# gchhablani/multilingual-image-captioning

Hardware: AMD Instinct MI355X
Metric: train images/sec, ViT-B/32+mBART-50 (bf16 train step, batch 64/GPU, 224x224, seq_len 64) (higher is better)
Workload: dtype bf16

## Files before the change

### include/mic_hip.h

```cpp
#ifndef MIC_HIP_H
#define MIC_HIP_H
#include <stdint.h>
#ifdef __cplusplus
extern "C" {
#endif

#define MIC_OK 0
#define MIC_EINVAL (-1)
#define MIC_ELAUNCH (-2)

#define MIC_BF16 0
#define MIC_F32 1
#define MIC_FP8 2
#define MIC_E4M3 0
#define MIC_E5M2 1

#define MIC_ACT_NONE 0
#define MIC_ACT_GELU_ERF 1
#define MIC_ACT_GELU_TANH 2
#define MIC_ACT_QUICK_GELU 3

int mic_version(void);
const char* mic_last_error(void);

// ... 125 lines not shown
int mic_ce_rows_tiles(int dtype, int rows, int V, const void* logits, int ld, const float* rowstat, int stat_ld,
                      const int32_t* labels, float* row_lse, float* row_loss, void* stream);
int mic_ce_reduce(int rows, const float* row_loss, const int32_t* mask, float* loss_out, float* denom_out,
                  void* stream);
int mic_ce_bwd(int dtype, int rows, int V, int Vpad, void* logits, int ld, const int32_t* labels,
               const int32_t* mask, float label_smoothing, const float* row_lse, const float* denom,
               float loss_scale, void* stream);
int mic_ce_bwd_q8(int rows, int V, int Vpad, const void* logits, int ld, const int32_t* labels, const int32_t* mask,
                  float label_smoothing, const float* row_lse, const float* denom, float loss_scale, const mic_fp8_out* q8,
                  float* colsum, float* label_coef, void* stream);
int mic_head_label_terms(int rows, int width, const int32_t* labels, const float* coef, const void* E, int lde, const void* h, int ldh,
                         float* dx_slab, int ldx, float* dE, int ldde, void* stream);
int mic_ce_bwd_t(int rows, int V, int Vpad, void* logits, int ld, const int32_t* labels, const int32_t* mask, float label_smoothing,
                 const float* row_lse, const float* denom, float loss_scale, void* dlogits_t, int ld_t, int rows_pad, float* colsum,
                 void* stream);
int mic_transpose_bf16(int rows, int rows_pad, int cols, const void* src, int ld_src, void* dst, int ld_dst, void* stream);

int mic_colsum(int dtype, int rows, int cols, const void* x, int ld, float* out, int accumulate, void* stream);
typedef struct { const void* x; float* out; int rows, cols, ld; } mic_colsum_item;
int mic_colsum_grouped(int dtype, const mic_colsum_item* items, int count, void* stream);
typedef struct { const void* x; float* out; const float* scale_inv; int rows, cols, ld, fmt; } mic_colsum_q8_item;
int mic_colsum_q8_grouped(const mic_colsum_q8_item* items, int count, void* stream);
int mic_dropout_mask(uint8_t* out, int64_t n, float p, uint32_t seed, void* stream);
int mic_cast(int src_dtype, int dst_dtype, const void* src, void* dst, int64_t n, void* stream);
int mic_zero(void* p, int64_t bytes, void* stream);
int mic_stream_create_cu_masked(int first_cu, int n_cus, void** stream);
int mic_stream_destroy(void* stream);
int mic_comm_emulate(const void* src, void* dst, int64_t bytes, float micros, int blocks, void* stream);
int mic_copy_rows(int dtype, int n, int width, const void* src, int ld_src, const int32_t* src_idx, void* dst, int ld_dst,
                  const int32_t* dst_idx, void* stream);
// ... 54 lines not shown
```

### multilingual-image-captioning_amd/_lib.py

```python
from __future__ import annotations

import ctypes as C
import os

_HERE = os.path.dirname(os.path.abspath(__file__))
LIB_PATH = os.path.join(_HERE, "libmic_hip.so")

MIC_BF16, MIC_F32, MIC_FP8 = 0, 1, 2
MIC_E4M3, MIC_E5M2 = 0, 1
ACT_NONE, ACT_GELU_ERF, ACT_GELU_TANH, ACT_QUICK_GELU = 0, 1, 2, 3
ACT_IDS = {"none": 0, None: 0, "gelu": 1, "erf": 1, "gelu_erf": 1, "tanh": 2, "gelu_tanh": 2, "gelu_new": 2, "quick_gelu": 3}


class MicError(RuntimeError):
    pass


class GemmArgs(C.Structure):
    _fields_ = [
        ("dtype", C.c_int), ("c_dtype", C.c_int), ("M", C.c_int), ("N", C.c_int), ("K", C.c_int),
        ("a_kmajor", C.c_int), ("b_kmajor", C.c_int),
        ("A", C.c_void_p), ("lda", C.c_int), ("B", C.c_void_p), ("ldb", C.c_int), ("C", C.c_void_p), ("ldc", C.c_int),
        ("bias", C.c_void_p), ("act", C.c_int), ("Zout", C.c_void_p), ("ldz", C.c_int), ("Zin", C.c_void_p),
        ("dact", C.c_int), ("R", C.c_void_p), ("ldr", C.c_int), ("accumulate", C.c_int), ("dropout_p", C.c_float),
# ... 84 lines not shown
    "mic_attn_decode": ([_i, _i, _i, _i, _i, _p, _i, _p, _p, _i, _p, _i, _p, _i, _p], C.c_int),
    "mic_kv_append": ([_i, _i, _i, _i, _i, _p, _i, _p, _i, _p, _p, _p], C.c_int),
    "mic_im2col": ([_i, _i, _i, _i, _p, _p, _i, _i, _p], C.c_int),
    "mic_vit_assemble": ([_i, _i, _i, _i, _p, _i, _p, _p, _p, _p], C.c_int),
    "mic_vit_assemble_bwd": ([_i, _i, _i, _i, _p, _p, _i, _p, _p, _p], C.c_int),
    "mic_embed_fwd": ([_i, _i, _i, _p, _p, _p, _p, _f, _p, _p], C.c_int),
    "mic_embed_bwd": ([_i, _i, _i, _p, _p, _p, _f, _p, _p, _p], C.c_int),
    "mic_embed_rows_add_det": ([_i, _i, _i, _i, _p, _p, _f, _p, _p, _p], C.c_int),
    "mic_embed_rows_add_det_ws": ([_i], C.c_int64),
    "mic_ce_rows": ([_i, _i, _i, _p, _i, _p, _p, _f, _p, _p, _p], C.c_int),
    "mic_ce_rows_tiles": ([_i, _i, _i, _p, _i, _p, _i, _p, _p, _p, _p], C.c_int),
    "mic_row_topk_tiles": ([_i, _i, _i, _p, _i, _p, _i, _i, _i, _i, _i, _p, _p, _p, _p], C.c_int),
    "mic_ce_reduce": ([_i, _p, _p, _p, _p, _p], C.c_int),
    "mic_ce_bwd": ([_i, _i, _i, _i, _p, _i, _p, _p, _f, _p, _p, _f, _p], C.c_int),
    "mic_ce_bwd_t": ([_i, _i, _i, _p, _i, _p, _p, _f, _p, _p, _f, _p, _i, _i, _p, _p], C.c_int),
    "mic_ce_bwd_q8": ([_i, _i, _i, _p, _i, _p, _p, _f, _p, _p, _f, C.POINTER(Fp8Out), _p, _p, _p], C.c_int),
    "mic_head_label_terms": ([_i, _i, _p, _p, _p, _i, _p, _i, _p, _i, _p, _i, _p], C.c_int),
    "mic_transpose_bf16": ([_i, _i, _i, _p, _i, _p, _i, _p], C.c_int),
    "mic_colsum": ([_i, _i, _i, _p, _i, _p, _i, _p], C.c_int),
    "mic_colsum_grouped": ([_i, C.POINTER(ColsumItem), _i, _p], C.c_int),
    "mic_dropout_mask": ([_p, _i64, _f, _u32, _p], C.c_int),
    "mic_cast": ([_i, _i, _p, _p, _i64, _p], C.c_int),
    "mic_zero": ([_p, _i64, _p], C.c_int),
    "mic_stream_create_cu_masked": ([_i, _i, C.POINTER(C.c_void_p)], C.c_int),
    "mic_stream_destroy": ([_p], C.c_int),
    "mic_copy_rows": ([_i, _i, _i, _p, _i, _p, _p, _i, _p, _p], C.c_int),
    "mic_cast2d": ([_i, _i, _i, _i, _p, _i, _p, _i, _p], C.c_int),
    "mic_adamw": ([_i64, _p, _p, _p, _p, _p, _p, C.c_double, C.c_double, C.c_double, C.c_double, _f, _p], C.c_int),
    "mic_adamw_rows": ([_i64, _i, _p, _i, _p, _p, _p, _p, _p, _p, C.c_double, C.c_double, C.c_double, C.c_double, _f, _p], C.c_int),
    "mic_row_flags": ([_p, _i, _p, _i, _p], C.c_int),
# ... 30 lines not shown
```

### multilingual-image-captioning_amd/csrc/elementwise.hip

```cpp
#include "common.h"
#include <stdarg.h>
#include <type_traits>

static thread_local char g_err[512] = "";
void mic_set_error(const char* fmt, ...) {
  va_list ap;
  va_start(ap, fmt);
  vsnprintf(g_err, sizeof(g_err), fmt, ap);
  va_end(ap);
}
extern "C" const char* mic_last_error(void) { return g_err; }
extern "C" int mic_version(void) { return 1; }

template <typename F>
static int dispatch_t(int dtype, F&& f) {
  if (dtype == MIC_BF16) f((uint16_t*)nullptr);
  else if (dtype == MIC_F32) f((float*)nullptr);
  else { mic_set_error("bad dtype %d", dtype); return MIC_EINVAL; }
  hipError_t e = hipGetLastError();
  if (e != hipSuccess) { mic_set_error("launch failed: %s", hipGetErrorString(e)); return MIC_ELAUNCH; }
  return MIC_OK;
}
#define TYPE_OF(tag) typename std::remove_pointer<decltype(tag)>::type

// ... 497 lines not shown
                          float loss_scale, void* stream) {
  MIC_CHECK(rows > 0 && V > 1 && Vpad >= V && Vpad % 8 == 0 && ld >= Vpad && logits && labels && mask && row_lse && denom, "mic_ce_bwd: bad args");
  return dispatch_t(dtype, [&](auto* tag) {
    using T = TYPE_OF(tag);
    hipLaunchKernelGGL(ce_bwd_kernel<T>, dim3(rows), dim3(256), 0, (hipStream_t)stream, V, Vpad, (T*)logits, ld, labels, mask, label_smoothing, row_lse, denom, loss_scale);
  });
}

struct TransposeArgs {
  const uint16_t* src; uint16_t* src_rw; int ld_src;
  uint16_t* dst; int ld_dst;
  int rows, cols;
  int V; const int32_t* labels; const int32_t* mask; float ls; const float* row_lse; const float* denom; float loss_scale;
  float* colsum;
};
template <int OP>
__global__ __launch_bounds__(256) void tile_transpose_kernel(TransposeArgs a) {
  __shared__ __attribute__((aligned(16))) char img[64 * 1024];
  const int tid = threadIdx.x, lane = tid & 63, wave = tid >> 6;
  const int c0 = blockIdx.x * 512, r0 = blockIdx.y * 64;
  const int col = c0 + lane * 8;
  const bool col_ok = col < a.cols;
  uint4 q[16];
#pragma unroll
  for (int rr = 0; rr < 16; ++rr) {
    const int row = r0 + wave * 16 + rr;
    q[rr] = make_uint4(0u, 0u, 0u, 0u);
    if (row < a.rows && col_ok) q[rr] = *reinterpret_cast<const uint4*>(a.src + (size_t)row * a.ld_src + col);
  }
  float inv_denom = 0.f;
  if constexpr (OP == 1) inv_denom = a.loss_scale / a.denom[0];
#pragma unroll
  for (int rr = 0; rr < 16; ++rr) {
// ... 63 lines not shown
}
extern "C" int mic_ce_bwd_t(int rows, int V, int Vpad, void* logits, int ld, const int32_t* labels, const int32_t* mask,
                            float label_smoothing, const float* row_lse, const float* denom, float loss_scale, void* dlogits_t,
                            int ld_t, int rows_pad, float* colsum, void* stream) {
  if (rows_pad <= 0) rows_pad = (rows + 63) / 64 * 64;
  MIC_CHECK(rows_pad >= rows && rows_pad % 64 == 0, "mic_ce_bwd_t: rows_pad >= rows, a multiple of 64");
  MIC_CHECK(rows > 0 && V > 1 && Vpad >= V && Vpad % 8 == 0 && ld >= Vpad && ld % 8 == 0 && logits && labels && mask && row_lse && denom && dlogits_t,
            "mic_ce_bwd_t: bad args");
  MIC_CHECK(ld_t >= rows_pad && ld_t % 8 == 0 && ((uintptr_t)logits & 15) == 0 && ((uintptr_t)dlogits_t & 15) == 0,
            "mic_ce_bwd_t: ld_t >= rows rounded up to 64, ld_t %% 8 == 0, 16-B aligned operands");
  TransposeArgs a{};
  a.src = (const uint16_t*)logits; a.src_rw = (uint16_t*)logits; a.ld_src = ld; a.dst = (uint16_t*)dlogits_t; a.ld_dst = ld_t;
  a.rows = rows; a.cols = Vpad; a.V = V; a.labels = labels; a.mask = mask; a.ls = label_smoothing; a.row_lse = row_lse; a.denom = denom;
  a.loss_scale = loss_scale; a.colsum = colsum;
  hipLaunchKernelGGL(tile_transpose_kernel<1>, dim3((Vpad + 511) / 512, rows_pad / 64), dim3(256), 0, (hipStream_t)stream, a);
  MIC_LAUNCH_CHECK();
  return MIC_OK;
}

struct CeQ8Args {
  const uint16_t* logits; int ld; int rows, V, Vpad;
  const int32_t* labels; const int32_t* mask; float ls; const float* row_lse; const float* denom; float loss_scale;
  float* colsum; uint8_t* q; int ldq; float* state; int fmt;
  float* label_coef;
};
constexpr int CEQ8_RG = 4;
__global__ __launch_bounds__(256) void ce_bwd_q8_kernel(CeQ8Args a) {
  __shared__ __attribute__((aligned(16))) float cs[4][512];
  const int tid = threadIdx.x, lane = tid & 63, wave = tid >> 6;
  const int c0 = blockIdx.x * 512;
// ... 488 lines not shown
```

### multilingual-image-captioning_amd/csrc/gemm.hip

```cpp
#include "gemm_common.h"

__global__ __launch_bounds__(256) void gemm_f32_kernel(const float* __restrict__ A, long sam, long sak,
                                                       const float* __restrict__ B, long sbk, long sbn, int M, int N,
                                                       int K, EpiArgs epi) {
  __shared__ float As[64][17];
  __shared__ float Bs[16][65];
  const int tid = threadIdx.x, lane = tid & 63, wave = tid >> 6;
  const int m0 = blockIdx.y * 64, n0 = blockIdx.x * 64;
  const int wr = wave >> 1, wc = wave & 1;
  f32x16 acc;
#pragma unroll
  for (int r = 0; r < 16; ++r) acc[r] = 0.0f;
  for (int k0 = 0; k0 < K; k0 += 16) {
#pragma unroll
    for (int i = 0; i < 4; ++i) {
      const int e = tid + i * 256;
      {
        int mm, kk;
        if (sak == 1) { mm = e >> 4; kk = e & 15; } else { kk = e >> 6; mm = e & 63; }
        const int gm = m0 + mm, gk = k0 + kk;
        As[mm][kk] = (gm < M && gk < K) ? A[gm * sam + gk * sak] : 0.0f;
      }
      {
        int nn, kk;
// ... 222 lines not shown
    if (c128 < c256) bm = 128;
  }
  const int force = sw.tile == 256 || sw.tile == 128 || sw.tile == 64 ? sw.tile : 0;
  if (force) bm = force;
  if (d.f8 && d.akm && bm < 128) bm = 128;
  if (c_q8 && bm == 256) bm = 128;
  if (rowstat) bm = 256;
  bool t192 = false;
  if (bm == 128 && sw.t192 && sw.tile == 0 && count == 1 && !d.f8 && !d.akm && args[0].split_k <= 1) {
    const long t128 = (long)((args[0].M + 127) / 128) * ((args[0].N + 127) / 128), t192n = (long)((args[0].M + 191) / 192) * ((args[0].N + 127) / 128);
    t192 = t128 > 2L * cus && t192n <= 2L * cus;
  }
  const bool nt1 = bm == 256 && !d.f8 && !d.akm && !d.bkm && count == 1;
  d.phased = nt1 && sw.phased != 0 && !rowsum;
  if (d.phased && sw.w4 && args[0].K >= 256 && args[0].K % 128 == 0) d.phased = 2;
  const int w4_epi = d.phased == 2 ? gemm_w4_takes(tab) : -1;
  const int d2_epi = sw.d2 && nt1 ? gemm_d2_takes(tab) : -1;
  if (d2_epi >= 0 && (sw.d2 == 2 || w4_epi >= 0) && (sw.d2 != 3 || tab.p[0].epi.rowstat)) d.family = GEMM_D2;
  else if (w4_epi >= 0) d.family = GEMM_W4;
  else if (bm == 256 && d.phased && tab.p[0].nsplit == 1) d.family = GEMM_PHASED;
  else d.family = bm == 256 ? GEMM_T256 : (t192 ? GEMM_T192 : (bm == 128 ? GEMM_T128 : GEMM_T64));
  d.tile_m = d.family == GEMM_T192 ? 192 : bm;
  d.tile_n = d.family == GEMM_D2 ? 128 : bm;
  d.epi = d.family == GEMM_D2 ? d2_epi : (d.family == GEMM_W4 ? w4_epi : 0);
  tile_table(tab, d.tile_m, d.tile_n);
  d.blocks = d.grid = tab.total_blocks;
  int kmin = 1 << 30;
  for (int i = 0; i < count; ++i) kmin = tab.p[i].K / 64 / tab.p[i].nsplit < kmin ? tab.p[i].K / 64 / tab.p[i].nsplit : kmin;
  d.kgroups = 1;
  d.per_cu = 1;
  if (d.family == GEMM_D2 || d.family == GEMM_T192) {
    d.per_cu = 2;
  } else if (d.family == GEMM_T256) {
    if (sw.persist && d.plain && d.blocks > cus) d.grid = cus;
  } else if (d.family == GEMM_T128) {
    const bool two = sw.kg128 >= 0 ? sw.kg128 == 2 : (d.blocks <= cus && kmin >= 8);
    d.kgroups = two ? 2 : 1;
    d.per_cu = two ? 1 : 2;
  } else if (d.family == GEMM_T64) {
    d.kgroups = d.blocks <= cus && kmin >= 16 ? 4 : (d.blocks <= 2 * cus && kmin >= 8 ? 2 : 1);
    if (sw.kg == 1 || sw.kg == 2 || sw.kg == 4) d.kgroups = sw.kg;
    d.per_cu = 4 / d.kgroups;
  }
  return d;
}

extern "C" int mic_gemm_plan(const mic_gemm_args* args, int count, mic_gemm_plan_info* out) {
  MIC_CHECK(args && out && count >= 1 && count <= MAX_PROBLEMS, "mic_gemm_plan: bad args (1..%d problems)", MAX_PROBLEMS);
// ... 62 lines not shown
```

### multilingual-image-captioning_amd/csrc/gemm_common.h

```cpp
#pragma once
#include "common.h"

#define MAX_PROBLEMS 8
#ifndef MIC_TINY_BELOW
#define MIC_TINY_BELOW 128
#endif

struct Problem {
  const uint16_t* A; const uint16_t* B;
  int lda, ldb, M, N, K;
  int tiles_m, tiles_n, block_begin, nsplit;
  float* a_rowsum; int rowsum_k;
  int k_valid;
  long long split_stride;
  const float* sa; const float* sb;
  EpiArgs epi;
};
struct LaunchTable { int count; int total_blocks; Problem p[MAX_PROBLEMS]; };
enum GemmFamily { GEMM_T64 = 0, GEMM_T128, GEMM_T192, GEMM_T256, GEMM_PHASED, GEMM_W4, GEMM_D2 };
struct GemmDecision {
  int family;
  int tile_m, tile_n;
  int kgroups, per_cu;
  int akm, bkm, f8;
  int plain;
  int epi;
  int blocks, grid;
  int phased;
};
void launch_gemm_phased(const LaunchTable& tab, const GemmDecision& d, hipStream_t s);
int gemm_w4_takes(const LaunchTable& tab);
void launch_gemm_w4(const LaunchTable& tab, const GemmDecision& d, hipStream_t s);
int gemm_d2_takes(const LaunchTable& tab);
void launch_gemm_d2(const LaunchTable& tab, const GemmDecision& d, hipStream_t s);
void launch_gemm_t256(const LaunchTable& tab, const GemmDecision& d, hipStream_t s);
void launch_gemm_t128(const LaunchTable& tab, const GemmDecision& d, hipStream_t s);
void launch_gemm_t192(const LaunchTable& tab, const GemmDecision& d, hipStream_t s);
void launch_gemm_t64(const LaunchTable& tab, const GemmDecision& d, hipStream_t s);

template <bool KMAJOR, int NWAVES, int BKT, int ROWS>
struct HalfStager {
  static_assert(ROWS == 128 || (ROWS == 64 && BKT == 64), "image = 128 rows (x) of BKT k, or 64 rows of 64 k");
  static constexpr int NINST = ROWS * BKT * 2 / 1024;
  static constexpr int PER = NINST / NWAVES;
  static_assert(PER >= 1, "too many waves for this image");
  static __device__ __forceinline__ void coords(int q, int lane, int& row, int& c) {
// ... 191 lines not shown
```

### multilingual-image-captioning_amd/csrc/gemm_w4.hip

```cpp
#include "gemm_common.h"
#ifdef MIC_TRACE_BLOCKS
__device__ unsigned long long* mic_trace_buf;
#define MIC_TRACE(SLOT) do { if (threadIdx.x == 0) mic_trace_buf[5 * blockIdx.x + (SLOT)] = wall_clock64(); } while (0)
#define MIC_TRACE_ID() do { if (threadIdx.x == 0) { unsigned hw_, xcc_; asm volatile("s_getreg_b32 %0, hwreg(HW_REG_HW_ID)" : "=s"(hw_)); \
  asm volatile("s_getreg_b32 %0, hwreg(HW_REG_XCC_ID)" : "=s"(xcc_)); mic_trace_buf[5 * blockIdx.x + 4] = ((unsigned long long)(xcc_ & 0xf) << 16) | (hw_ & 0xffff); } } while (0)
#else
#define MIC_TRACE(SLOT) do { } while (0)
#define MIC_TRACE_ID() do { } while (0)
#endif

namespace {

constexpr int W4_BK = 64, W4_HIMG = 128 * W4_BK * 2, W4_SLOT = 4 * W4_HIMG;

__device__ __forceinline__ uint32_t w4_source(int ld, int x0, int lim, int q, int lane) {
  const int R = q * 8 + (lane >> 3), c = (lane & 7) ^ ((R >> 1) & 7);
  int gx = x0 + R;
  gx = gx < lim ? gx : lim - 1;
  return ((uint32_t)gx * (uint32_t)ld + (uint32_t)(c * 8)) * 2u;
}

constexpr int W4_EP = 132;
template <bool STATS, bool LNF>
__device__ __forceinline__ void w4_epilogue_lean(f32x16 (&acc)[4][4], const Problem& P, char* smem, int mw, int nw, int wave, int lane) {
// ... 114 lines not shown
      const int row = it * 2 + urow;
      const int m = mw + p * 32 + row;
      const float4 v = *reinterpret_cast<const float4*>(Cw + row * W4_EP + c4);
      if (m < M && n < N) {
        float* dst = C + (size_t)m * ldc + n;
        if (nfull) *reinterpret_cast<float4*>(dst) = v;
        else {
          const float x[4] = {v.x, v.y, v.z, v.w};
          for (int i = 0; i < N - n && i < 4; ++i) dst[i] = x[i];
        }
      }
    }
  }
}

template <int EPI>
__global__ __launch_bounds__(256) void gemm_w4_kernel(LaunchTable tab) {
  constexpr int WM = 128, WN = 128, WNW = 2, AI = 4, NJ = 4, BM = 256, BN = 256;
  extern __shared__ __attribute__((aligned(16))) char smem[];
  const int tid = threadIdx.x, lane = tid & 63, wave = __builtin_amdgcn_readfirstlane(tid >> 6);
  int lid;
  {
    const int bid = blockIdx.x, nwg = tab.total_blocks;
    const int xcd = bid & 7, q = nwg >> 3, r = nwg & 7;
    lid = (xcd < r ? xcd * (q + 1) : r * (q + 1) + (xcd - r) * q) + (bid >> 3);
  }
  const Problem& P = tab.p[0];
  MIC_TRACE(0);
  MIC_TRACE_ID();
  int tile = lid, split = 0;
  if (P.nsplit > 1) {
    const int T = P.tiles_m * P.tiles_n;
    if ((P.nsplit & 7) == 0) {
      const int S = P.nsplit >> 3, j = blockIdx.x >> 3;
      split = (blockIdx.x & 7) * S + j / T;
// ... 95 lines not shown
    asm volatile("s_waitcnt vmcnt(0)" ::: "memory");
  }
  __syncthreads();
  MIC_TRACE(2);
  if (live) {
    if constexpr (EPI == 8) w4_epilogue_f32(acc, P, smem, m0 + wr * WM, n0 + wc * WN, split, wave, lane);
    else w4_epilogue_lean<(EPI & 1) != 0, (EPI & 4) != 0>(acc, P, smem, m0 + wr * WM, n0 + wc * WN, wave, lane);
  }
#ifdef MIC_TRACE_BLOCKS
  asm volatile("s_waitcnt vmcnt(0)" ::: "memory");
#endif
  MIC_TRACE(3);
}

template <int EPI>
void launch_w4(const LaunchTable& tab, hipStream_t s) {
  constexpr int lds = 2 * W4_SLOT;
  static bool attr_set_dev[64] = {};
  int dev_ = 0;
  (void)hipGetDevice(&dev_);
  bool& attr_set = attr_set_dev[dev_ & 63];
  if (!attr_set) {
    hipFuncSetAttribute(reinterpret_cast<const void*>(&gemm_w4_kernel<EPI>), hipFuncAttributeMaxDynamicSharedMemorySize, lds);
    attr_set = true;
  }
  hipLaunchKernelGGL((gemm_w4_kernel<EPI>), dim3(tab.total_blocks), dim3(256), lds, s, tab);
}

}

int gemm_w4_takes(const LaunchTable& tab) {
  if (tab.count != 1) return -1;
  const Problem& p = tab.p[0];
  const EpiArgs& e = p.epi;
  const long long lim = 0x7fffffffLL;
  if ((long long)p.M * p.lda * 2 >= lim || (long long)p.N * p.ldb * 2 >= lim) return -1;
  if (p.K < 256 || p.K % 128 != 0 || e.R || e.drop_thr || e.rowsum2 || e.act || e.Zout || e.dact || e.accumulate) return -1;
  if (((uintptr_t)e.C & 15) != 0) return -1;
  if (e.c_f32)
    return !e.rowstat && !e.ln_stats && (p.nsplit == 1 || p.split_stride > 0) && p.K / 64 / p.nsplit >= 2 ? 8 : -1;
  if (!(p.nsplit == 1 && (e.ldc & 7) == 0 && (!e.ln_stats || p.N % 8 == 0))) return -1;
  return 2 + (e.rowstat ? 1 : 0) + (e.ln_stats ? 4 : 0);
}
void launch_gemm_w4(const LaunchTable& tab, const GemmDecision& d, hipStream_t s) {
  switch (d.epi) {
    case 8: launch_w4<8>(tab, s); break;
    case 2: launch_w4<2>(tab, s); break;
    case 3: launch_w4<3>(tab, s); break;
    case 6: launch_w4<6>(tab, s); break;
    default: launch_w4<7>(tab, s); break;
  }
}
```

### multilingual-image-captioning_amd/engine.py

```python
from __future__ import annotations

import math
from typing import Dict, Optional

import torch

from . import _lib as L
from . import ops
from .params import ParamStore, _rup

ROWPAD = 128


def _mix(seed: int, site: int) -> int:
    x = (seed * 0x9E3779B1 + site * 0x85EBCA6B + 0x27D4EB2F) & 0xFFFFFFFF
    x ^= x >> 15
    x = (x * 0x2C1B3C6D) & 0xFFFFFFFF
    x ^= x >> 12
    return x & 0xFFFFFFFF


class Engine:
    def __init__(self, store: ParamStore):
        self.P = store
# ... 12 lines not shown
        self._cs_queue = []
        self.on_free = []
        self.fp8 = False
        import os
        self.use_head_stats = os.environ.get("MIC_HEAD_STATS", "1") != "0"
        self.grad_progress = None
        self.on_embed_rows = None
        self.dw_overlap = self.dev.type == "cuda" and os.environ.get("MIC_DW_OVERLAP", "1") != "0"
        self.decode_ln_fold = self.dev.type == "cuda" and os.environ.get("MIC_DECODE_LNFOLD", "1") != "0"
        self._ckv_hoist = os.environ.get("MIC_CKV_HOIST", "1") != "0"
        self._lnf = {}
        self._lnf_version = -1
        self._dw_stream = None
        import os as _os
        self.head_nt = _os.environ.get("MIC_HEAD_NT", "1") != "0"
        self.ln_partials = _os.environ.get("MIC_LN_PARTIALS", "1") != "0"
        self._lnp_queue = []
        self._head_nt_state = None
        self.fp8_head = 0
        self._head8_state = None
        self._head_x8 = None
        self._ET_version, self._ET_event = -1, None
        self._dw_events = []
        self.dw_every = int(os.environ.get("MIC_DW_EVERY", "0"))
        self.dw_late_flush = os.environ.get("MIC_DW_LATE_FLUSH", "1") != "0"
        self._dw_side = False
        self._ckv_block_name = None

    FP8_KINDS = ("qkv", "cq", "ckv", "fc1", "fc2")

# ... 686 lines not shown
        self._head_nt_state = None
        h8s, self._head8_state = self._head8_state, None
        if h8s is not None:
            x8 = self._head_x8 or self._quant(hf, Mh, d, "head.x", "head.x", torch.float8_e4m3fn)
            ops.gemm(h8s[0], x8[0], P.g("shared"), P.Vpad, d, _rup(Mh, 128), a_kmajor=True, b_kmajor=True, k_valid=Mh,
                     a_scale_inv=h8s[1][1:], b_scale_inv=x8[1][1:])
            tiles = ((Mh + 255) // 256) * ((d + 255) // 256)
            nsp = max(1, min(ops.get_cu_budget() // tiles, P.Vpad // 128 // 2))
            slab_rows = _rup(Mh, 256)
            cap_rows = max(_rup(Mcap, 256), (256 // max(1, (d + 255) // 256)) * 256) + _rup(Mcap, 256)
            d32 = self.buf("db.dhf32", cap_rows, d, torch.float32)
            assert (nsp + 1) * slab_rows <= d32.shape[0], (nsp, slab_rows, d32.shape)
            ops.head_label_terms(h8s[3], h8s[2], P.w("shared"), hf, d32[nsp * slab_rows:], P.g("shared"), Mh, d)
        elif nt is not None:
            dT, Kp = nt
            hfT = self.buf("d.hfT", d, dT.shape[1])
            ops.transpose_bf16(hf, hfT, Mh, d, rows_pad=Kp)
            ops.gemm(dT, hfT, P.g("shared"), P.Vpad, d, Kp)
        elif self.dt == torch.bfloat16:
            ops.zero(P.g("flb"))
            ops.gemm(dlogits, hf, P.g("shared"), P.Vpad, d, Mhp, a_kmajor=True, b_kmajor=True, a_rowsum=P.g("flb"), rowsum_k=Mh)
        else:
            ops.colsum(dlogits, P.g("flb"), Mh, P.Vpad, dlogits.stride(0))
            ops.gemm(dlogits, hf, P.g("shared"), P.Vpad, d, Mhp, a_kmajor=True, b_kmajor=True)
        self._done("shared")
        dhc = dhf if (rows is None or pack is not None) else self.buf("db.dhfc", Mcap, d)
        if h8s is not None:
            _, ET8, wst = self._w8["shared"]
            self._w8_wait()
            slab = slab_rows * d
            ops.gemm(h8s[0], ET8, d32, Mh, d, P.Vpad, split_k=nsp, split_stride=slab if nsp > 1 else 0, a_scale_inv=h8s[1][1:], b_scale_inv=wst[1:])
            ops.sum_slabs(d32, nsp + 1, slab, dhc, Mh, d, d32.stride(0), dhc.stride(0))
        elif nt is not None:
# ... 200 lines not shown
            ops.ce_rows(logits, logits.stride(0), P.V, labels, mask, label_smoothing, lse, rl, M)
        ops.ce_reduce(rl, mask, loss, denom, M)
        if backward and self._head8():
            ops.zero(P.g("flb"))
            q = self.buf("head.dl.q8", logits.shape[0], P.Vpad, torch.float8_e5m2)
            st = self.vec("head.dl.state", 2)
            coef = self.vec("head.dl.coef", _rup(logits.shape[0], ROWPAD))
            ops.ce_bwd_q8(logits, logits.stride(0), P.V, P.Vpad, labels, mask, label_smoothing, lse, denom, M, ops.fp8_out(q, st), colsum=P.g("flb"),
                          label_coef=coef)
            self._head8_state = (q, st, coef, labels)
            self._head_nt_state = None
        elif backward:
            kcap = self._head_nt_kcap(logits)
            if kcap:
                Kp = _rup(M, 128)
                dT = self.buf("d.dlogitsT", P.Vpad, kcap)
                ops.zero(P.g("flb"))
                ops.ce_bwd_t(logits, logits.stride(0), P.V, P.Vpad, labels, mask, label_smoothing, lse, denom, M, dT, rows_pad=Kp, colsum=P.g("flb"))
                self._head_nt_state = (dT, Kp)
            else:
                ops.ce_bwd(logits, logits.stride(0), P.V, P.Vpad, labels, mask, label_smoothing, lse, denom, M)
                self._head_nt_state = None
        return loss

    def _head_nt_kcap(self, logits) -> int:
        P = self.P
        if not self.head_nt or self.dt != torch.bfloat16 or P.Vpad < 16384 or P.d % 128 != 0 or self._head8():
            return 0
        kcap = _rup(logits.shape[0], 128)
        return kcap if P.Vpad * kcap * 2 < 0x7fffffff and logits.shape[0] * logits.stride(0) * 2 < 0x7fffffff else 0

    def shared_T(self):
        P = self.P
        ET = self.buf("w.sharedT", P.d, P.Vpad)
# ... 102 lines not shown
```

### multilingual-image-captioning_amd/ops.py

```python
from __future__ import annotations

import ctypes as C
from typing import Optional

import torch

from . import _lib as L


_FP8 = {torch.float8_e4m3fn: L.MIC_E4M3, torch.float8_e5m2: L.MIC_E5M2}


def _dt(t_or_dtype) -> int:
    d = t_or_dtype.dtype if isinstance(t_or_dtype, torch.Tensor) else t_or_dtype
    if d == torch.bfloat16:
        return L.MIC_BF16
    if d == torch.float32:
        return L.MIC_F32
    if d in _FP8:
        return L.MIC_FP8
    raise L.MicError(f"unsupported dtype {d}")


def _p(t: Optional[torch.Tensor]):
# ... 287 lines not shown
def ce_bwd(logits, ld, V, Vpad, labels, mask, ls, row_lse, denom, rows, loss_scale=1.0):
    L.check(L.lib().mic_ce_bwd(_dt(logits), rows, V, Vpad, _p(logits), ld, _p(labels), _p(mask), float(ls), _p(row_lse), _p(denom),
                               float(loss_scale), _stream()), "mic_ce_bwd")


def ce_bwd_q8(logits, ld, V, Vpad, labels, mask, ls, row_lse, denom, rows, q8, colsum=None, label_coef=None, loss_scale=1.0):
    L.check(L.lib().mic_ce_bwd_q8(rows, V, Vpad, _p(logits), ld, _p(labels), _p(mask), float(ls), _p(row_lse), _p(denom), float(loss_scale),
                                  C.byref(q8), _p(colsum), _p(label_coef), _stream()), "mic_ce_bwd_q8")


def head_label_terms(labels, coef, E, h, dx_slab, dE, rows, width):
    L.check(L.lib().mic_head_label_terms(rows, width, _p(labels), _p(coef), _p(E), E.stride(0), _p(h), h.stride(0), _p(dx_slab), dx_slab.stride(0),
                                         _p(dE), dE.stride(0), _stream()), "mic_head_label_terms")


def ce_bwd_t(logits, ld, V, Vpad, labels, mask, ls, row_lse, denom, rows, dlogits_t, rows_pad=0, colsum=None, loss_scale=1.0):
    L.check(L.lib().mic_ce_bwd_t(rows, V, Vpad, _p(logits), ld, _p(labels), _p(mask), float(ls), _p(row_lse), _p(denom), float(loss_scale),
                                 _p(dlogits_t), dlogits_t.stride(0), int(rows_pad), _p(colsum), _stream()), "mic_ce_bwd_t")


def transpose_bf16(src, dst, rows, cols, rows_pad=0):
    L.check(L.lib().mic_transpose_bf16(int(rows), int(rows_pad), int(cols), _p(src), src.stride(0), _p(dst), dst.stride(0), _stream()),
            "mic_transpose_bf16")
    return dst


def colsum(x, out, rows, cols, ld, accumulate=False):
    L.check(L.lib().mic_colsum(_dt(x), rows, cols, _p(x), ld, _p(out), int(accumulate), _stream()), "mic_colsum")


# ... 137 lines not shown
```

Before: 3553.

## Compute head dE with K-major W4 GEMM instead of transposing dlogits

```diff
diff --git a/include/mic_hip.h b/include/mic_hip.h
--- a/include/mic_hip.h
+++ b/include/mic_hip.h
@@ -163,6 +163,8 @@
 int mic_ce_bwd_t(int rows, int V, int Vpad, void* logits, int ld, const int32_t* labels, const int32_t* mask, float label_smoothing,
                  const float* row_lse, const float* denom, float loss_scale, void* dlogits_t, int ld_t, int rows_pad, float* colsum,
                  void* stream);
+int mic_ce_bwd_cs(int rows, int V, int Vpad, void* logits, int ld, const int32_t* labels, const int32_t* mask, float label_smoothing,
+                  const float* row_lse, const float* denom, float loss_scale, float* colsum, void* stream);
 int mic_transpose_bf16(int rows, int rows_pad, int cols, const void* src, int ld_src, void* dst, int ld_dst, void* stream);
 
 int mic_colsum(int dtype, int rows, int cols, const void* x, int ld, float* out, int accumulate, void* stream);
diff --git a/multilingual-image-captioning_amd/_lib.py b/multilingual-image-captioning_amd/_lib.py
--- a/multilingual-image-captioning_amd/_lib.py
+++ b/multilingual-image-captioning_amd/_lib.py
@@ -122,6 +122,7 @@
     "mic_ce_reduce": ([_i, _p, _p, _p, _p, _p], C.c_int),
     "mic_ce_bwd": ([_i, _i, _i, _i, _p, _i, _p, _p, _f, _p, _p, _f, _p], C.c_int),
     "mic_ce_bwd_t": ([_i, _i, _i, _p, _i, _p, _p, _f, _p, _p, _f, _p, _i, _i, _p, _p], C.c_int),
+    "mic_ce_bwd_cs": ([_i, _i, _i, _p, _i, _p, _p, _f, _p, _p, _f, _p, _p], C.c_int),
     "mic_ce_bwd_q8": ([_i, _i, _i, _p, _i, _p, _p, _f, _p, _p, _f, C.POINTER(Fp8Out), _p, _p, _p], C.c_int),
     "mic_head_label_terms": ([_i, _i, _p, _p, _p, _i, _p, _i, _p, _i, _p, _i, _p], C.c_int),
     "mic_transpose_bf16": ([_i, _i, _i, _p, _i, _p, _i, _p], C.c_int),
diff --git a/multilingual-image-captioning_amd/csrc/elementwise.hip b/multilingual-image-captioning_amd/csrc/elementwise.hip
--- a/multilingual-image-captioning_amd/csrc/elementwise.hip
+++ b/multilingual-image-captioning_amd/csrc/elementwise.hip
@@ -535,9 +535,71 @@
   int V; const int32_t* labels; const int32_t* mask; float ls; const float* row_lse; const float* denom; float loss_scale;
   float* colsum;
 };
+constexpr int CECS_RG = 4;
+__device__ __forceinline__ void ce_bwd_colsum_rows(const TransposeArgs& a, char* img) {
+  float (*cs)[512] = reinterpret_cast<float (*)[512]>(img);
+  const int tid = threadIdx.x, lane = tid & 63, wave = tid >> 6;
+  const int c0 = blockIdx.x * 512;
+  const int col = c0 + lane * 8;
+  const bool col_ok = col < a.cols;
+  const float inv_denom = a.loss_scale / a.denom[0];
+  const float conf = 1.0f - a.ls, low = a.ls > 0.f ? a.ls / (float)(a.V - 1) : 0.f;
+  float csum[8] = {0.f, 0.f, 0.f, 0.f, 0.f, 0.f, 0.f, 0.f};
+  for (int rg = 0; rg < CECS_RG; ++rg) {
+    const int r0 = (blockIdx.y * CECS_RG + rg) * 64;
+    if (r0 >= a.rows) break;
+    uint4 q[16];
+#pragma unroll
+    for (int rr = 0; rr < 16; ++rr) {
+      const int row = r0 + wave * 16 + rr;
+      q[rr] = make_uint4(0u, 0u, 0u, 0u);
+      if (row < a.rows && col_ok) q[rr] = *reinterpret_cast<const uint4*>(a.src + (size_t)row * a.ld_src + col);
+    }
+#pragma unroll
+    for (int rr = 0; rr < 16; ++rr) {
+      const int row = r0 + wave * 16 + rr;
+      if (row < a.rows && col_ok) {
+        const float w = a.mask[row] ? inv_denom : 0.f;
+        const float lse = a.row_lse[row];
+        const int label = a.labels[row];
+        const uint32_t wd[4] = {q[rr].x, q[rr].y, q[rr].z, q[rr].w};
+        float o[8];
+#pragma unroll
+        for (int i = 0; i < 8; ++i) {
+          const float x = __uint_as_float((i & 1) ? (wd[i >> 1] & 0xffff0000u) : (wd[i >> 1] << 16));
+          const int c = col + i;
+          o[i] = c < a.V ? w * (__expf(x - lse) - (c == label ? conf : low)) : 0.f;
+        }
+        uint4 u;
+        u.x = f2bf_pk(o[0], o[1]); u.y = f2bf_pk(o[2], o[3]); u.z = f2bf_pk(o[4], o[5]); u.w = f2bf_pk(o[6], o[7]);
+        *reinterpret_cast<uint4*>(a.src_rw + (size_t)row * a.ld_src + col) = u;
+        const uint32_t ws[4] = {u.x, u.y, u.z, u.w};
+#pragma unroll
+        for (int i = 0; i < 8; ++i) csum[i] += __uint_as_float((i & 1) ? (ws[i >> 1] & 0xffff0000u) : (ws[i >> 1] << 16));
+      }
+    }
+  }
+  if (a.colsum != nullptr) {
+    *reinterpret_cast<float4*>(&cs[wave][lane * 8]) = make_float4(csum[0], csum[1], csum[2], csum[3]);
+    *reinterpret_cast<float4*>(&cs[wave][lane * 8 + 4]) = make_float4(csum[4], csum[5], csum[6], csum[7]);
+    __syncthreads();
+#pragma unroll
+    for (int h = 0; h < 2; ++h) {
+      const int c = tid + h * 256;
+      const float s4 = (cs[0][c] + cs[1][c]) + (cs[2][c] + cs[3][c]);
+      if (c0 + c < a.cols && s4 != 0.f) atomicAdd(a.colsum + c0 + c, s4);
+    }
+  }
+}
 template <int OP>
 __global__ __launch_bounds__(256) void tile_transpose_kernel(TransposeArgs a) {
   __shared__ __attribute__((aligned(16))) char img[64 * 1024];
+  if constexpr (OP == 1) {
+    if (a.dst == nullptr) {
+      ce_bwd_colsum_rows(a, img);
+      return;
+    }
+  }
   const int tid = threadIdx.x, lane = tid & 63, wave = tid >> 6;
   const int c0 = blockIdx.x * 512, r0 = blockIdx.y * 64;
   const int col = c0 + lane * 8;
@@ -631,6 +693,21 @@
   a.rows = rows; a.cols = Vpad; a.V = V; a.labels = labels; a.mask = mask; a.ls = label_smoothing; a.row_lse = row_lse; a.denom = denom;
   a.loss_scale = loss_scale; a.colsum = colsum;
   hipLaunchKernelGGL(tile_transpose_kernel<1>, dim3((Vpad + 511) / 512, rows_pad / 64), dim3(256), 0, (hipStream_t)stream, a);
+  MIC_LAUNCH_CHECK();
+  return MIC_OK;
+}
+
+extern "C" int mic_ce_bwd_cs(int rows, int V, int Vpad, void* logits, int ld, const int32_t* labels, const int32_t* mask,
+                             float label_smoothing, const float* row_lse, const float* denom, float loss_scale, float* colsum,
+                             void* stream) {
+  MIC_CHECK(rows > 0 && V > 1 && Vpad >= V && Vpad % 8 == 0 && ld >= Vpad && ld % 8 == 0 && logits && labels && mask && row_lse && denom,
+            "mic_ce_bwd_cs: bad args");
+  MIC_CHECK(((uintptr_t)logits & 15) == 0, "mic_ce_bwd_cs: 16-B aligned bf16 logits");
+  TransposeArgs a{};
+  a.src = (const uint16_t*)logits; a.src_rw = (uint16_t*)logits; a.ld_src = ld; a.dst = nullptr; a.ld_dst = 0;
+  a.rows = rows; a.cols = Vpad; a.V = V; a.labels = labels; a.mask = mask; a.ls = label_smoothing; a.row_lse = row_lse; a.denom = denom;
+  a.loss_scale = loss_scale; a.colsum = colsum;
+  hipLaunchKernelGGL(tile_transpose_kernel<1>, dim3((Vpad + 511) / 512, (rows + 64 * CECS_RG - 1) / (64 * CECS_RG)), dim3(256), 0, (hipStream_t)stream, a);
   MIC_LAUNCH_CHECK();
   return MIC_OK;
 }
diff --git a/multilingual-image-captioning_amd/csrc/gemm.hip b/multilingual-image-captioning_amd/csrc/gemm.hip
--- a/multilingual-image-captioning_amd/csrc/gemm.hip
+++ b/multilingual-image-captioning_amd/csrc/gemm.hip
@@ -260,7 +260,8 @@
   const bool nt1 = bm == 256 && !d.f8 && !d.akm && !d.bkm && count == 1;
   d.phased = nt1 && sw.phased != 0 && !rowsum;
   if (d.phased && sw.w4 && args[0].K >= 256 && args[0].K % 128 == 0) d.phased = 2;
-  const int w4_epi = d.phased == 2 ? gemm_w4_takes(tab) : -1;
+  const bool tn1 = bm == 256 && !d.f8 && d.akm && d.bkm && count == 1 && sw.w4 != 0 && !rowsum;
+  const int w4_epi = d.phased == 2 ? gemm_w4_takes(tab) : (tn1 ? gemm_w4_takes(tab, true) : -1);
   const int d2_epi = sw.d2 && nt1 ? gemm_d2_takes(tab) : -1;
   if (d2_epi >= 0 && (sw.d2 == 2 || w4_epi >= 0) && (sw.d2 != 3 || tab.p[0].epi.rowstat)) d.family = GEMM_D2;
   else if (w4_epi >= 0) d.family = GEMM_W4;
@@ -277,7 +278,7 @@
   d.per_cu = 1;
   if (d.family == GEMM_D2 || d.family == GEMM_T192) {
     d.per_cu = 2;
-  } else if (d.family == GEMM_T256) {
+  } else if (d.family == GEMM_T256 || (d.family == GEMM_W4 && d.akm)) {
     if (sw.persist && d.plain && d.blocks > cus) d.grid = cus;
   } else if (d.family == GEMM_T128) {
     const bool two = sw.kg128 >= 0 ? sw.kg128 == 2 : (d.blocks <= cus && kmin >= 8);
diff --git a/multilingual-image-captioning_amd/csrc/gemm_common.h b/multilingual-image-captioning_amd/csrc/gemm_common.h
--- a/multilingual-image-captioning_amd/csrc/gemm_common.h
+++ b/multilingual-image-captioning_amd/csrc/gemm_common.h
@@ -29,7 +29,7 @@
   int phased;
 };
 void launch_gemm_phased(const LaunchTable& tab, const GemmDecision& d, hipStream_t s);
-int gemm_w4_takes(const LaunchTable& tab);
+int gemm_w4_takes(const LaunchTable& tab, bool kmajor = false);
 void launch_gemm_w4(const LaunchTable& tab, const GemmDecision& d, hipStream_t s);
 int gemm_d2_takes(const LaunchTable& tab);
 void launch_gemm_d2(const LaunchTable& tab, const GemmDecision& d, hipStream_t s);
diff --git a/multilingual-image-captioning_amd/csrc/gemm_w4.hip b/multilingual-image-captioning_amd/csrc/gemm_w4.hip
--- a/multilingual-image-captioning_amd/csrc/gemm_w4.hip
+++ b/multilingual-image-captioning_amd/csrc/gemm_w4.hip
@@ -152,11 +152,157 @@
   }
 }
 
+__device__ __forceinline__ uint32_t w4_source_kmajor(int ld, int x0, int lim, int q, int lane) {
+  const int k = q * 4 + (lane >> 4), c = (lane & 15) ^ ((k & 3) << 2);
+  int gx = x0 + c * 8;
+  gx = gx < lim ? gx : 0;
+  return ((uint32_t)k * (uint32_t)ld + (uint32_t)gx) * 2u;
+}
+template <int KK>
+__device__ __forceinline__ bf16x8 w4_read_frag_kmajor(const char* lds_tile, int xb, int lane) {
+  const int g = lane >> 4, p = lane & 15;
+  const int x = xb + 16 * (g & 1) + (p & 3) * 4;
+  const int k = 8 * (g >> 1) + (p >> 2);
+  const uint32_t a = (uint32_t)(uintptr_t)LDS_PTR(char, lds_tile + k * 256 + ((((x >> 3) ^ ((k & 3) << 2)) << 4) | ((x & 7) << 1)));
+  s16x4 lo, hi;
+  asm volatile("ds_read_b64_tr_b16 %0, %1 offset:%2" : "=v"(lo) : "v"(a), "n"(KK * 16 * 256));
+  asm volatile("ds_read_b64_tr_b16 %0, %1 offset:%2" : "=v"(hi) : "v"(a), "n"(KK * 16 * 256 + 4 * 256));
+  s16x8 r = {lo[0], lo[1], lo[2], lo[3], hi[0], hi[1], hi[2], hi[3]};
+  return __builtin_bit_cast(bf16x8, r);
+}
+#define W4_BARRIER()                       \
+  do {                                     \
+    __builtin_amdgcn_sched_barrier(0);     \
+    __builtin_amdgcn_s_barrier();          \
+    __builtin_amdgcn_sched_barrier(0);     \
+  } while (0)
+__device__ __forceinline__ void w4_kmajor_tiles(const LaunchTable& tab, char* smem, int wave) {
+  constexpr int WM = 128, WN = 128, AI = 4, NJ = 4, BM = 256, BN = 256;
+  const Problem& P = tab.p[0];
+  const int wr = wave >> 1, wc = wave & 1;
+  const int M = P.M, N = P.N, lda = P.lda, ldb = P.ldb;
+  const int nk = P.K / 64;
+  const int kv = P.k_valid;
+  const int nwg = tab.total_blocks;
+  const char* fa_ = smem + wr * W4_HIMG;
+  const char* fb_ = smem + (2 + wc) * W4_HIMG;
+  const uint32_t lds0 = (uint32_t)(uintptr_t)LDS_PTR(char, smem) + (uint32_t)wave * 4096u;
+  const __amdgpu_buffer_rsrc_t rA = __builtin_amdgcn_make_buffer_rsrc((void*)P.A, 0, max(((kv - 1) * lda + M) * 2, 0), 0x00020000);
+  const __amdgpu_buffer_rsrc_t rB = __builtin_amdgcn_make_buffer_rsrc((void*)P.B, 0, max(((kv - 1) * ldb + N) * 2, 0), 0x00020000);
+  const uint32_t stepA = 128u * (uint32_t)lda, stepB = 128u * (uint32_t)ldb;
+  for (int v = blockIdx.x; v < nwg; v += gridDim.x) {
+    int ln;
+    asm volatile("v_mbcnt_lo_u32_b32 %0, -1, 0\n\tv_mbcnt_hi_u32_b32 %0, -1, %0" : "=v"(ln));
+    int tm, tn;
+    {
+      const int xcd = v & 7, q = nwg >> 3, r = nwg & 7;
+      tile_coords((xcd < r ? xcd * (q + 1) : r * (q + 1) + (xcd - r) * q) + (v >> 3), P.tiles_m, P.tiles_n, tm, tn);
+    }
+    const int m0 = tm * BM, n0 = tn * BN;
+    f32x16 acc[AI][NJ];
+#pragma unroll
+    for (int i = 0; i < AI; ++i)
+#pragma unroll
+      for (int j = 0; j < NJ; ++j)
+#pragma unroll
+        for (int r = 0; r < 16; ++r) acc[i][j][r] = 0.0f;
+    uint32_t go[16];
+#pragma unroll
+    for (int h = 0; h < 4; ++h)
+#pragma unroll
+      for (int i = 0; i < 4; ++i)
+        go[h * 4 + i] = h < 2 ? w4_source_kmajor(lda, m0 + h * 128, M, wave * 4 + i, ln) : w4_source_kmajor(ldb, n0 + (h - 2) * 128, N, wave * 4 + i, ln);
+    bf16x8 fa[AI][4], fb[NJ][4];
+#define W4K_DMA(SLOT, Q)                                                                                                       \
+  do {                                                                                                                         \
+    __builtin_amdgcn_raw_ptr_buffer_load_lds((Q) < 8 ? rA : rB,                                                                \
+                                             (__attribute__((address_space(3))) void*)(lb_ + (SLOT) * W4_SLOT + ((Q) >> 2) * W4_HIMG + ((Q) & 3) * 1024), \
+                                             16, go[Q], 0, 0, 0);                                                              \
+    go[Q] += (Q) < 8 ? stepA : stepB;                                                                                          \
+  } while (0)
+#define W4K_TILE(C)                                                                                                            \
+  do {                                                                                                                         \
+    uint32_t lb_ = lds0;     \
+    asm volatile("" : "+s"(lb_));                                                                                              \
+    _Pragma("unroll") for (int g_ = 0; g_ < 64; ++g_) {                                                                        \
+      if (g_ == 16) {                                                                                                          \
+        asm volatile("s_waitcnt vmcnt(0) lgkmcnt(0)" ::: "memory");                                                            \
+        W4_BARRIER();                                                                                                          \
+      }                                                                                                                        \
+      acc[(g_ & 15) >> 2][g_ & 3] = __builtin_amdgcn_mfma_f32_32x32x16_bf16(fa[(g_ & 15) >> 2][g_ >> 4], fb[g_ & 3][g_ >> 4],  \
+                                                                           acc[(g_ & 15) >> 2][g_ & 3], 0, 0, 0);             \
+      const int q_ = g_ >> 4, x_ = g_ & 15;                                                                                    \
+      const int rk_ = (q_ + 3) & 3, rs_ = q_ == 0 ? (C) : 1 - (C);                                                             \
+      if (x_ == 0 && q_ != 1) asm volatile("s_waitcnt lgkmcnt(0)" ::: "memory");           \
+      if (x_ < 8) {                                                                                                            \
+        const char* im_ = (x_ < 4 ? fa_ : fb_) + rs_ * W4_SLOT;                                                                \
+        bf16x8& f_ = x_ < 4 ? fa[x_ & 3][rk_] : fb[x_ & 3][rk_];                                                               \
+        if (rk_ == 0) f_ = w4_read_frag_kmajor<0>(im_, (x_ & 3) * 32, ln);                                                     \
+        else if (rk_ == 1) f_ = w4_read_frag_kmajor<1>(im_, (x_ & 3) * 32, ln);                                                \
+        else if (rk_ == 2) f_ = w4_read_frag_kmajor<2>(im_, (x_ & 3) * 32, ln);                                                \
+        else f_ = w4_read_frag_kmajor<3>(im_, (x_ & 3) * 32, ln);                                                              \
+      }                                                                                                                        \
+      if ((q_ == 1 || q_ == 2) && (x_ & 1) == 1) W4K_DMA(C, (q_ - 1) * 8 + (x_ >> 1));                                         \
+      __builtin_amdgcn_sched_barrier(0);                                                                                       \
+    }                                                                                                                          \
+  } while (0)
+    const bool live = m0 + wr * WM < M;
+    {
+      uint32_t lb_ = lds0;
+      asm volatile("" : "+s"(lb_));
+#pragma unroll
+      for (int q = 0; q < 16; ++q) W4K_DMA(0, q);
+#pragma unroll
+      for (int q = 0; q < 16; ++q) W4K_DMA(1, q);
+      asm volatile("s_waitcnt vmcnt(16)" ::: "memory");
+      W4_BARRIER();
+#pragma unroll
+      for (int x = 0; x < 4; ++x) {
+        fa[x][0] = w4_read_frag_kmajor<0>(fa_, x * 32, ln); fb[x][0] = w4_read_frag_kmajor<0>(fb_, x * 32, ln);
+        fa[x][1] = w4_read_frag_kmajor<1>(fa_, x * 32, ln); fb[x][1] = w4_read_frag_kmajor<1>(fb_, x * 32, ln);
+        fa[x][2] = w4_read_frag_kmajor<2>(fa_, x * 32, ln); fb[x][2] = w4_read_frag_kmajor<2>(fb_, x * 32, ln);
+      }
+      asm volatile("s_waitcnt lgkmcnt(0)" ::: "memory");
+      __builtin_amdgcn_sched_barrier(0);
+      if (live) {
+        int t = 0;
+        do {
+          W4K_TILE(0);
+          W4K_TILE(1);
+          t += 2;
+        } while (t < nk);
+      } else {
+        int t = 0;
+        do {
+          asm volatile("s_waitcnt vmcnt(0)" ::: "memory");
+          W4_BARRIER();
+          asm volatile("" : "+s"(lb_));
+#pragma unroll
+          for (int q = 0; q < 16; ++q) W4K_DMA(t & 1, q);
+        } while (++t < nk);
+      }
+      asm volatile("s_waitcnt vmcnt(0) lgkmcnt(0)" ::: "memory");
+    }
+    __syncthreads();
+    if (live) w4_epilogue_f32(acc, P, smem, m0 + wr * WM, n0 + wc * WN, 0, wave, ln);
+    __syncthreads();
+  }
+}
+#undef W4K_DMA
+#undef W4K_TILE
+
 template <int EPI>
 __global__ __launch_bounds__(256) void gemm_w4_kernel(LaunchTable tab) {
   constexpr int WM = 128, WN = 128, WNW = 2, AI = 4, NJ = 4, BM = 256, BN = 256;
   extern __shared__ __attribute__((aligned(16))) char smem[];
-  const int tid = threadIdx.x, lane = tid & 63, wave = __builtin_amdgcn_readfirstlane(tid >> 6);
+  const int wave = __builtin_amdgcn_readfirstlane(threadIdx.x >> 6);
+  if constexpr (EPI == 8) {
+    if (tab.p[0].k_valid != 0x7fffffff) {
+      w4_kmajor_tiles(tab, smem, wave);
+      return;
+    }
+  }
+  const int lane = __builtin_amdgcn_mbcnt_hi(~0u, __builtin_amdgcn_mbcnt_lo(~0u, 0u));
   int lid;
   {
     const int bid = blockIdx.x, nwg = tab.total_blocks;
@@ -282,7 +428,7 @@
 }
 
 template <int EPI>
-void launch_w4(const LaunchTable& tab, hipStream_t s) {
+void launch_w4(const LaunchTable& tab, int grid, hipStream_t s) {
   constexpr int lds = 2 * W4_SLOT;
   static bool attr_set_dev[64] = {};
   int dev_ = 0;
@@ -292,30 +438,40 @@
     hipFuncSetAttribute(reinterpret_cast<const void*>(&gemm_w4_kernel<EPI>), hipFuncAttributeMaxDynamicSharedMemorySize, lds);
     attr_set = true;
   }
-  hipLaunchKernelGGL((gemm_w4_kernel<EPI>), dim3(tab.total_blocks), dim3(256), lds, s, tab);
-}
-
-}
-
-int gemm_w4_takes(const LaunchTable& tab) {
+  hipLaunchKernelGGL((gemm_w4_kernel<EPI>), dim3(grid), dim3(256), lds, s, tab);
+}
+
+}
+
+int gemm_w4_takes(const LaunchTable& tab, bool kmajor) {
   if (tab.count != 1) return -1;
   const Problem& p = tab.p[0];
   const EpiArgs& e = p.epi;
   const long long lim = 0x7fffffffLL;
-  if ((long long)p.M * p.lda * 2 >= lim || (long long)p.N * p.ldb * 2 >= lim) return -1;
+  if (kmajor ? ((long long)p.K * p.lda * 2 >= lim || (long long)p.K * p.ldb * 2 >= lim) : ((long long)p.M * p.lda * 2 >= lim || (long long)p.N * p.ldb * 2 >= lim)) return -1;
   if (p.K < 256 || p.K % 128 != 0 || e.R || e.drop_thr || e.rowsum2 || e.act || e.Zout || e.dact || e.accumulate) return -1;
   if (((uintptr_t)e.C & 15) != 0) return -1;
+  if (kmajor) {
+    if ((((uintptr_t)p.A | (uintptr_t)p.B) & 15) != 0 || ((p.lda | p.ldb | p.M | p.N) & 7) != 0 || p.lda < p.M || p.ldb < p.N) return -1;
+    return e.c_f32 && !e.rowstat && !e.ln_stats && p.nsplit == 1 && !p.a_rowsum ? 8 : -1;
+  }
   if (e.c_f32)
     return !e.rowstat && !e.ln_stats && (p.nsplit == 1 || p.split_stride > 0) && p.K / 64 / p.nsplit >= 2 ? 8 : -1;
   if (!(p.nsplit == 1 && (e.ldc & 7) == 0 && (!e.ln_stats || p.N % 8 == 0))) return -1;
   return 2 + (e.rowstat ? 1 : 0) + (e.ln_stats ? 4 : 0);
 }
 void launch_gemm_w4(const LaunchTable& tab, const GemmDecision& d, hipStream_t s) {
+  if (d.akm) {
+    LaunchTable t = tab;
+    t.p[0].k_valid = t.p[0].k_valid < t.p[0].K ? t.p[0].k_valid : t.p[0].K;
+    launch_w4<8>(t, d.grid, s);
+    return;
+  }
   switch (d.epi) {
-    case 8: launch_w4<8>(tab, s); break;
-    case 2: launch_w4<2>(tab, s); break;
-    case 3: launch_w4<3>(tab, s); break;
-    case 6: launch_w4<6>(tab, s); break;
-    default: launch_w4<7>(tab, s); break;
-  }
-}
+    case 8: launch_w4<8>(tab, d.grid, s); break;
+    case 2: launch_w4<2>(tab, d.grid, s); break;
+    case 3: launch_w4<3>(tab, d.grid, s); break;
+    case 6: launch_w4<6>(tab, d.grid, s); break;
+    default: launch_w4<7>(tab, d.grid, s); break;
+  }
+}
diff --git a/multilingual-image-captioning_amd/engine.py b/multilingual-image-captioning_amd/engine.py
--- a/multilingual-image-captioning_amd/engine.py
+++ b/multilingual-image-captioning_amd/engine.py
@@ -50,6 +50,7 @@
         self._dw_stream = None
         import os as _os
         self.head_nt = _os.environ.get("MIC_HEAD_NT", "1") != "0"
+        self.head_de_kmajor = _os.environ.get("MIC_HEAD_DE_KMAJOR", "1") != "0"
         self.ln_partials = _os.environ.get("MIC_LN_PARTIALS", "1") != "0"
         self._lnp_queue = []
         self._head_nt_state = None
@@ -766,9 +767,12 @@
             ops.head_label_terms(h8s[3], h8s[2], P.w("shared"), hf, d32[nsp * slab_rows:], P.g("shared"), Mh, d)
         elif nt is not None:
             dT, Kp = nt
-            hfT = self.buf("d.hfT", d, dT.shape[1])
-            ops.transpose_bf16(hf, hfT, Mh, d, rows_pad=Kp)
-            ops.gemm(dT, hfT, P.g("shared"), P.Vpad, d, Kp)
+            if dT is None:
+                ops.gemm(dlogits, hf, P.g("shared"), P.Vpad, d, Kp, a_kmajor=True, b_kmajor=True, k_valid=Mh)
+            else:
+                hfT = self.buf("d.hfT", d, dT.shape[1])
+                ops.transpose_bf16(hf, hfT, Mh, d, rows_pad=Kp)
+                ops.gemm(dT, hfT, P.g("shared"), P.Vpad, d, Kp)
         elif self.dt == torch.bfloat16:
             ops.zero(P.g("flb"))
             ops.gemm(dlogits, hf, P.g("shared"), P.Vpad, d, Mhp, a_kmajor=True, b_kmajor=True, a_rowsum=P.g("flb"), rowsum_k=Mh)
@@ -999,10 +1003,14 @@
             kcap = self._head_nt_kcap(logits)
             if kcap:
                 Kp = _rup(M, 128)
-                dT = self.buf("d.dlogitsT", P.Vpad, kcap)
                 ops.zero(P.g("flb"))
-                ops.ce_bwd_t(logits, logits.stride(0), P.V, P.Vpad, labels, mask, label_smoothing, lse, denom, M, dT, rows_pad=Kp, colsum=P.g("flb"))
-                self._head_nt_state = (dT, Kp)
+                if self.head_de_kmajor:
+                    ops.ce_bwd_cs(logits, logits.stride(0), P.V, P.Vpad, labels, mask, label_smoothing, lse, denom, M, colsum=P.g("flb"))
+                    self._head_nt_state = (None, Kp)
+                else:
+                    dT = self.buf("d.dlogitsT", P.Vpad, kcap)
+                    ops.ce_bwd_t(logits, logits.stride(0), P.V, P.Vpad, labels, mask, label_smoothing, lse, denom, M, dT, rows_pad=Kp, colsum=P.g("flb"))
+                    self._head_nt_state = (dT, Kp)
             else:
                 ops.ce_bwd(logits, logits.stride(0), P.V, P.Vpad, labels, mask, label_smoothing, lse, denom, M)
                 self._head_nt_state = None
diff --git a/multilingual-image-captioning_amd/ops.py b/multilingual-image-captioning_amd/ops.py
--- a/multilingual-image-captioning_amd/ops.py
+++ b/multilingual-image-captioning_amd/ops.py
@@ -325,6 +325,11 @@
                                          _p(dE), dE.stride(0), _stream()), "mic_head_label_terms")
 
 
+def ce_bwd_cs(logits, ld, V, Vpad, labels, mask, ls, row_lse, denom, rows, colsum=None, loss_scale=1.0):
+    L.check(L.lib().mic_ce_bwd_cs(rows, V, Vpad, _p(logits), ld, _p(labels), _p(mask), float(ls), _p(row_lse), _p(denom), float(loss_scale),
+                                  _p(colsum), _stream()), "mic_ce_bwd_cs")
+
+
 def ce_bwd_t(logits, ld, V, Vpad, labels, mask, ls, row_lse, denom, rows, dlogits_t, rows_pad=0, colsum=None, loss_scale=1.0):
     L.check(L.lib().mic_ce_bwd_t(rows, V, Vpad, _p(logits), ld, _p(labels), _p(mask), float(ls), _p(row_lse), _p(denom), float(loss_scale),
                                  _p(dlogits_t), dlogits_t.stride(0), int(rows_pad), _p(colsum), _stream()), "mic_ce_bwd_t")
```

Result: no change. 3552, median of 4 (-0.0%).
